# mazouziwissem/improving_yolov8_CBAM_SwinBlock

Hardware: AMD Instinct MI355X
Metric: images/sec fwd+bwd YOLOv8s-CBAM-Swin bs=32 640x640 (higher is better)
Workload: dtype bf16; 1 GPU; yolov8s.yaml (nc=1) forward + v8 loss + backward + clip + SGD-nesterov + EMA step, bs=32/GPU 640x640 (CBAM + 2x SwinBlock + SPPF5 + SPPF7); global_batch=32, imgsz=640, parallelism=dp1

## Files before the change

### improving_yolov8_cbam_swinblock_amd/csrc/common.h

```cpp
#pragma once
#include <hip/hip_runtime.h>
#include <stdint.h>
#include <stdio.h>

#include "../../include/ymi.h"

typedef __bf16 bf16_t;
typedef __attribute__((ext_vector_type(8))) __bf16 bf16x8;
typedef __attribute__((ext_vector_type(4))) __bf16 bf16x4;
typedef __attribute__((ext_vector_type(4))) float f32x4;
typedef __attribute__((ext_vector_type(2))) float f32x2;
typedef __attribute__((ext_vector_type(4))) uint32_t u32x4;
typedef __attribute__((ext_vector_type(2))) uint32_t u32x2;

typedef const __attribute__((address_space(1))) void* gptr_t;
typedef __attribute__((address_space(3))) void* lptr_t;

#define YMI_WAVE 64

void ymi_set_error(const char* fmt, ...);
#define YMI_CHECK_ARG(cond, ...)          \
    do {                                  \
        if (!(cond)) {                    \
            ymi_set_error(__VA_ARGS__);   \
            return YMI_EINVAL;            \
        }                                 \
    } while (0)
#define YMI_CHECK_LAUNCH(what)                                                   \
    do {                                                                         \
        hipError_t e_ = hipGetLastError();                                       \
        if (e_ != hipSuccess) {                                                  \
            ymi_set_error("%s: launch failed: %s", what, hipGetErrorString(e_)); \
            return YMI_ELAUNCH;                                                  \
        }                                                                        \
    } while (0)

static inline bool ymi_tensor_ok(const ymi_tensor* t) {
    return t && t->data && t->n > 0 && t->h > 0 && t->w > 0 && t->c > 0 && t->ld >= t->c && (t->dtype == YMI_F32 || t->dtype == YMI_BF16);
}
static inline int64_t ymi_pixels(const ymi_tensor* t) { return t->n * t->h * t->w; }
static inline int ymi_stat_fixed_point_shift(int64_t count) {
    int lg = 0;
    while (((int64_t)1 << lg) < count) ++lg;
    const int sh = 37 - lg;
    return sh < 8 ? 8 : sh > 40 ? 40 : sh;
}
static inline size_t ymi_esize(int dtype) { return dtype == YMI_BF16 ? 2 : 4; }
static inline bool ymi_same_shape(const ymi_tensor* a, const ymi_tensor* b) {
    return a->n == b->n && a->h == b->h && a->w == b->w && a->c == b->c;
}
enum YmiOpt {
    OPT_EW_PPT,
    OPT_EW_CAP,
    OPT_RED_CAP,
    OPT_XCD_SHIFT,
    OPT_ATTN_TILED,
    OPT_WGRAD_BLOCKS,
    OPT_WGRAD_BLOCKS128,
    OPT_IGEMM_TILE_BM,
    OPT_IGEMM_TILE_BN,
    OPT_BN_TAIL,
    OPT_WGRAD_PATCH,
    OPT_COUNT
};
int ymi_opt(int id);
static inline int ew_ppt() { return ymi_opt(OPT_EW_PPT); }
static inline int ew_cap() { return ymi_opt(OPT_EW_CAP); }
const void* ymi_zero_page();

template <typename T> struct ElemTraits;
template <> struct ElemTraits<float> {
    static constexpr int CH = 4;
    static constexpr int DT = YMI_F32;
};
template <> struct ElemTraits<bf16_t> {
    static constexpr int CH = 8;
    static constexpr int DT = YMI_BF16;
};

__device__ __forceinline__ float to_f32(float v) { return v; }
__device__ __forceinline__ float to_f32(bf16_t v) { return (float)v; }
template <typename T> __device__ __forceinline__ T from_f32(float v);
template <> __device__ __forceinline__ float from_f32<float>(float v) { return v; }
template <> __device__ __forceinline__ bf16_t from_f32<bf16_t>(float v) { return (bf16_t)v; }

template <typename T, int G> struct Pack;
template <> struct Pack<float, 4> {
    static __device__ __forceinline__ void load(const float* p, float (&v)[4]) {
        f32x4 t = *reinterpret_cast<const f32x4*>(p);
        v[0] = t[0]; v[1] = t[1]; v[2] = t[2]; v[3] = t[3];
    }
    static __device__ __forceinline__ void store(float* p, const float (&v)[4]) {
        f32x4 t = {v[0], v[1], v[2], v[3]};
        *reinterpret_cast<f32x4*>(p) = t;
    }
};
template <> struct Pack<bf16_t, 4> {
    static __device__ __forceinline__ void load(const bf16_t* p, float (&v)[4]) {
        bf16x4 t = *reinterpret_cast<const bf16x4*>(p);
        v[0] = (float)t[0]; v[1] = (float)t[1]; v[2] = (float)t[2]; v[3] = (float)t[3];
    }
    static __device__ __forceinline__ void store(bf16_t* p, const float (&v)[4]) {
        bf16x4 t = {(bf16_t)v[0], (bf16_t)v[1], (bf16_t)v[2], (bf16_t)v[3]};
        *reinterpret_cast<bf16x4*>(p) = t;
    }
};
template <> struct Pack<bf16_t, 8> {
    static __device__ __forceinline__ void load(const bf16_t* p, float (&v)[8]) {
        bf16x8 t = *reinterpret_cast<const bf16x8*>(p);
#pragma unroll
        for (int i = 0; i < 8; ++i) v[i] = (float)t[i];
    }
    static __device__ __forceinline__ void store(bf16_t* p, const float (&v)[8]) {
        bf16x8 t;
#pragma unroll
        for (int i = 0; i < 8; ++i) t[i] = (bf16_t)v[i];
        *reinterpret_cast<bf16x8*>(p) = t;
    }
};

template <typename T> struct Raw4;
template <> struct Raw4<bf16_t> {
    typedef bf16x4 type;
    static __device__ __forceinline__ void to_f32(const bf16x4& r, float (&v)[4]) {
#pragma unroll
        for (int i = 0; i < 4; ++i) v[i] = (float)r[i];
    }
};
template <> struct Raw4<float> {
    typedef f32x4 type;
    static __device__ __forceinline__ void to_f32(const f32x4& r, float (&v)[4]) {
#pragma unroll
        for (int i = 0; i < 4; ++i) v[i] = r[i];
    }
};

__host__ __device__ __forceinline__ int64_t ymi_xcd_span(int64_t P) { return (((P + 63) >> 6) + 7) >> 3 << 6; }
struct XcdRange {
    int64_t lo, hi;
    int bi, nbx;
};
int64_t ymi_xcd_span_arg(int64_t P);
__device__ __forceinline__ XcdRange xcd_range(int64_t P, int64_t span_arg) {
    const int id = blockIdx.x, x = ((id & 7) + (int)(span_arg >> 56)) & 7;
    const int64_t span = span_arg & ((1ll << 56) - 1);
// ... 220 lines not shown
```

### improving_yolov8_cbam_swinblock_amd/csrc/first_conv.hip

```cpp
#include "common.h"

namespace {

constexpr int FC_TH = 8, FC_TW = 64;
constexpr int FC_PR = 2 * FC_TH + 1;
constexpr int FC_ROWB = (2 * FC_TW + 2) * 8;
constexpr int FC_WG_TILES = 4;

enum { FC_STATS = 0, FC_APPLY = 1, FC_BWD_REDUCE = 2, FC_BWD_WGRAD = 3 };

struct FirstConvArgs {
    const float* img;
    const float* w;
    void* x4;
    void* out;
    int64_t ldout;
    float* partials;
    const float* v0;
    const float* v1;
    const float* v2;
    const float* v3;
    float* slab;
    int act;
    int N, C, H, W, Ho, Wo;
    int tiles_h, tiles_w, total;
};

template <int CTRL> __device__ __forceinline__ float fc_dpp_add(float v) {
    return v + __builtin_bit_cast(float, __builtin_amdgcn_update_dpp(0, __builtin_bit_cast(int, v), CTRL, 0xF, 0xF, true));
}
__device__ __forceinline__ float fc_row16_sum(float v) {
    v = fc_dpp_add<0xB1>(v);
    v = fc_dpp_add<0x4E>(v);
    v = fc_dpp_add<0x141>(v);
    v = fc_dpp_add<0x140>(v);
    return v;
}
__device__ __forceinline__ float fc_act(float x, int act) { return act == YMI_ACT_SILU ? silu_f(x) : x; }
__device__ __forceinline__ float fc_act_grad(float x, int act) { return act == YMI_ACT_SILU ? silu_grad_f(x) : 1.0f; }
__device__ __forceinline__ uint32_t fc_pack2(float lo, float hi) {
    typedef __attribute__((ext_vector_type(2))) __bf16 bf16x2;
    const bf16x2 v = {(bf16_t)lo, (bf16_t)hi};
    return __builtin_bit_cast(uint32_t, v);
}

template <int SW> __device__ __forceinline__ int fc_swz(int row) { return SW == 2 ? ((row >> 3) & 1) : (((row >> 1) & 1) | (((row >> 3) & 1) << 1)); }
template <int SW> __device__ __forceinline__ bf16x8 fc_tr_load(const char* img, int rowb, int c0, int lane) {
    typedef __attribute__((ext_vector_type(4))) short s16x4;
    typedef __attribute__((ext_vector_type(8))) short s16x8;
    const int g = lane >> 4, i = lane & 15, q = i >> 2, p = i & 3;
    const int r_lo = 8 * g + q, r_hi = r_lo + 4;
    const int u = (c0 >> 2) + p;
    const int u_lo = u ^ (fc_swz<SW>(r_lo) << 2), u_hi = u ^ (fc_swz<SW>(r_hi) << 2);
    const s16x4 lo = __builtin_amdgcn_ds_read_tr16_b64_v4i16((__attribute__((address_space(3))) s16x4*)(img + r_lo * rowb + u_lo * 8));
    const s16x4 hi = __builtin_amdgcn_ds_read_tr16_b64_v4i16((__attribute__((address_space(3))) s16x4*)(img + r_hi * rowb + u_hi * 8));
    const s16x8 v = {lo[0], lo[1], lo[2], lo[3], hi[0], hi[1], hi[2], hi[3]};
    return __builtin_bit_cast(bf16x8, v);
}

__device__ __forceinline__ void fc_patch_from_image(const FirstConvArgs& a, char* patch, int n, int oh0, int ow0, int tid) {
    const float* src = a.img + (int64_t)n * a.C * a.H * a.W;
    const int64_t plane = (int64_t)a.H * a.W;
    const int ih0 = 2 * oh0 - 1;
    constexpr int ITEMS = FC_PR * (2 * FC_TW / 4);
    constexpr int PASSES = (ITEMS + 255) / 256;
    f32x4 v[PASSES][3];
#pragma unroll
    for (int p = 0; p < PASSES; ++p) {
        const int it = tid + 256 * p;
        const int r = it / (2 * FC_TW / 4), g = it % (2 * FC_TW / 4);
        const int ih = ih0 + r, iw = 2 * ow0 + 4 * g;
        const bool ok = it < ITEMS && (unsigned)ih < (unsigned)a.H && iw < a.W;
#pragma unroll
        for (int c = 0; c < 3; ++c) v[p][c] = (ok && c < a.C) ? *reinterpret_cast<const f32x4*>(src + c * plane + (int64_t)ih * a.W + iw) : f32x4{0.f, 0.f, 0.f, 0.f};
    }
    float halo = 0.f;
    const int hr = tid / 4, hc = tid % 4;
    if (tid < FC_PR * 4) {
        const int ih = ih0 + hr, iw = 2 * ow0 - 1;
        if (hc < a.C && (unsigned)ih < (unsigned)a.H && iw >= 0) halo = src[hc * plane + (int64_t)ih * a.W + iw];
    }
#pragma unroll
    for (int p = 0; p < PASSES; ++p) {
        const int it = tid + 256 * p;
        if (it < ITEMS) {
            const int r = it / (2 * FC_TW / 4), g = it % (2 * FC_TW / 4);
            char* dst = patch + r * FC_ROWB + (4 * g + 2) * 8;
            *reinterpret_cast<u32x4*>(dst) = u32x4{fc_pack2(v[p][0][0], v[p][1][0]), fc_pack2(v[p][2][0], 0.f), fc_pack2(v[p][0][1], v[p][1][1]), fc_pack2(v[p][2][1], 0.f)};
            *reinterpret_cast<u32x4*>(dst + 16) = u32x4{fc_pack2(v[p][0][2], v[p][1][2]), fc_pack2(v[p][2][2], 0.f), fc_pack2(v[p][0][3], v[p][1][3]), fc_pack2(v[p][2][3], 0.f)};
        }
    }
    if (tid < FC_PR * 4) *reinterpret_cast<bf16_t*>(patch + hr * FC_ROWB + 1 * 8 + hc * 2) = (bf16_t)halo;
    if (a.C == 4) {
        __syncthreads();
        for (int e = tid; e < FC_PR * 2 * FC_TW; e += 256) {
            const int r = e / (2 * FC_TW), cc = e % (2 * FC_TW);
            const int ih = ih0 + r, iw = 2 * ow0 + cc;
            if ((unsigned)ih < (unsigned)a.H && iw < a.W) *reinterpret_cast<bf16_t*>(patch + r * FC_ROWB + (cc + 2) * 8 + 6) = (bf16_t)src[3 * plane + (int64_t)ih * a.W + iw];
        }
    }
    __syncthreads();
    bf16_t* x4 = reinterpret_cast<bf16_t*>(a.x4);
#pragma unroll 4
    for (int e = tid; e < 2 * FC_TH * FC_TW; e += 256) {
        const int r = e / FC_TW, cc = 2 * (e - r * FC_TW);
        const int ih = 2 * oh0 + r, iw = 2 * ow0 + cc;
        if (ih < a.H && iw < a.W) *reinterpret_cast<u32x4*>(x4 + (((int64_t)n * a.H + ih) * a.W + iw) * 4) = *reinterpret_cast<const u32x4*>(patch + (r + 1) * FC_ROWB + (cc + 2) * 8);
    }
}
__device__ __forceinline__ void fc_patch_from_x4(const FirstConvArgs& a, char* patch, int n, int oh0, int ow0, int tid) {
    const bf16_t* x4 = reinterpret_cast<const bf16_t*>(a.x4);
    const int ih0 = 2 * oh0 - 1;
    constexpr int ITEMS = FC_PR * FC_TW;
    constexpr int PASSES = (ITEMS + 255) / 256;
    u32x4 v[PASSES];
#pragma unroll
    for (int p = 0; p < PASSES; ++p) {
        const int it = tid + 256 * p;
        const int r = it / FC_TW, g = it % FC_TW;
        const int ih = ih0 + r, iw = 2 * ow0 + 2 * g;
        const bool ok = it < ITEMS && (unsigned)ih < (unsigned)a.H && iw < a.W;
        v[p] = ok ? *reinterpret_cast<const u32x4*>(x4 + (((int64_t)n * a.H + ih) * a.W + iw) * 4) : u32x4{0u, 0u, 0u, 0u};
    }
    u32x2 halo = u32x2{0u, 0u};
    if (tid < FC_PR) {
        const int ih = ih0 + tid, iw = 2 * ow0 - 1;
        if ((unsigned)ih < (unsigned)a.H && iw >= 0) halo = *reinterpret_cast<const u32x2*>(x4 + (((int64_t)n * a.H + ih) * a.W + iw) * 4);
    }
#pragma unroll
    for (int p = 0; p < PASSES; ++p) {
        const int it = tid + 256 * p;
        if (it < ITEMS) *reinterpret_cast<u32x4*>(patch + (it / FC_TW) * FC_ROWB + (2 * (it % FC_TW) + 2) * 8) = v[p];
    }
    if (tid < FC_PR) *reinterpret_cast<u32x2*>(patch + tid * FC_ROWB + 8) = halo;
    __syncthreads();
}

template <int NCT>
__device__ __forceinline__ void fc_conv_group(const char* patch, int ohl, int mt, int l15, int l4, const bf16x8 (&wf)[NCT][2], f32x4 (&acc)[NCT]) {
    const int owl = mt * 16 + l15;
    const int q0 = 2 * l4, q1 = 2 * l4 + 1;
    const u32x2 lo0 = *reinterpret_cast<const u32x2*>(patch + (2 * ohl + q0 / 3) * FC_ROWB + (2 * owl + q0 % 3 + 1) * 8);
    const u32x2 hi0 = *reinterpret_cast<const u32x2*>(patch + (2 * ohl + q1 / 3) * FC_ROWB + (2 * owl + q1 % 3 + 1) * 8);
    u32x2 lo1 = u32x2{0u, 0u};
    if (l4 == 0) lo1 = *reinterpret_cast<const u32x2*>(patch + (2 * ohl + 2) * FC_ROWB + (2 * owl + 2 + 1) * 8);
    const bf16x8 x0 = __builtin_bit_cast(bf16x8, u32x4{lo0[0], lo0[1], hi0[0], hi0[1]});
    const bf16x8 x1 = __builtin_bit_cast(bf16x8, u32x4{lo1[0], lo1[1], 0u, 0u});
#pragma unroll
    for (int ct = 0; ct < NCT; ++ct) {
        acc[ct] = __builtin_amdgcn_mfma_f32_16x16x32_bf16(wf[ct][0], x0, f32x4{0.f, 0.f, 0.f, 0.f}, 0, 0, 0);
        acc[ct] = __builtin_amdgcn_mfma_f32_16x16x32_bf16(wf[ct][1], x1, acc[ct], 0, 0, 0);
    }
}

template <int CO, int MODE>
__global__ __launch_bounds__(256, 4) void first_conv_kernel(FirstConvArgs a) {
    constexpr int NCT = CO / 16;
    constexpr int OUTB = FC_TW * CO * 2;
    constexpr int CPP = CO / 8;
    constexpr int DROWB = CO <= 32 ? 64 : 128, DSW = CO <= 32 ? 2 : 0;
    constexpr int STAGEB = MODE == FC_BWD_WGRAD ? FC_TW * DROWB : OUTB;
    __shared__ __attribute__((aligned(16))) char patch[FC_PR * FC_ROWB];
    __shared__ __attribute__((aligned(16))) char stage[(MODE == FC_APPLY || MODE == FC_BWD_WGRAD) ? 4 * STAGEB : 16];
    __shared__ __attribute__((aligned(16))) bf16_t wtab[CO * 64];
    __shared__ __attribute__((aligned(16))) float ctab[5 * CO];
    __shared__ float red[(MODE == FC_BWD_WGRAD) ? 48 * CO : 4 * 2 * CO];
    const int tid = threadIdx.x, lane = tid & 63, wave = tid >> 6;
    const int l15 = lane & 15, l4 = lane >> 4;

#pragma unroll
    for (int i = 0; i < CO * 64 / 256; ++i) {
        const int e = tid + 256 * i, co = e >> 6, k = e & 63, q = k >> 2, c = k & 3;
        wtab[e] = (bf16_t)((q < 9 && c < a.C) ? a.w[(co * a.C + c) * 9 + q] : 0.f);
    }
    if (tid < CO) {
        float c0 = 0.f, c1 = 0.f, c2 = 0.f, c3 = 0.f, c4 = 0.f;
        if constexpr (MODE == FC_APPLY) {
            c0 = a.v0[tid];
            c1 = a.v1[tid];
        } else if constexpr (MODE == FC_BWD_REDUCE) {
            const float g = a.v0 ? a.v0[tid] : 1.f, bb = a.v1 ? a.v1[tid] : 0.f, mu = a.v2[tid], iv = a.v3[tid];
            c0 = iv;
            c1 = -mu * iv;
            c2 = g;
            c3 = bb;
        } else if constexpr (MODE == FC_BWD_WGRAD) {
            c0 = a.v0[tid];
            c1 = a.v0[CO + tid];
            c2 = a.v0[2 * CO + tid];
            c3 = a.v0[3 * CO + tid];
            c4 = a.v0[4 * CO + tid];
        }
        ctab[tid] = c0; ctab[CO + tid] = c1; ctab[2 * CO + tid] = c2; ctab[3 * CO + tid] = c3; ctab[4 * CO + tid] = c4;
    }
    __syncthreads();
    bf16x8 wf[NCT][2];
#pragma unroll
    for (int ct = 0; ct < NCT; ++ct)
#pragma unroll
        for (int h = 0; h < 2; ++h) wf[ct][h] = *reinterpret_cast<const bf16x8*>(wtab + (ct * 16 + l15) * 64 + 32 * h + 8 * l4);

    float s1[NCT][4], s2[NCT][4];
#pragma unroll
    for (int ct = 0; ct < NCT; ++ct)
#pragma unroll
        for (int r = 0; r < 4; ++r) s1[ct][r] = s2[ct][r] = 0.f;
    f32x4 dwa[3][NCT];
#pragma unroll
    for (int kt = 0; kt < 3; ++kt)
#pragma unroll
        for (int ct = 0; ct < NCT; ++ct) dwa[kt][ct] = f32x4{0.f, 0.f, 0.f, 0.f};

    char* my = stage + ((MODE == FC_APPLY || MODE == FC_BWD_WGRAD) ? wave * STAGEB : 0);
    constexpr int TILES = MODE == FC_BWD_WGRAD ? FC_WG_TILES : 1;
    const int wg_unit = xcd_unit(blockIdx.x, gridDim.x);
#pragma unroll 1
    for (int ti = 0; ti < TILES; ++ti) {
        const int unit = wg_unit * TILES + ti;
        if (unit >= a.total) break;
        const int tw = unit % a.tiles_w;
        const int t2 = unit / a.tiles_w;
        const int th = t2 % a.tiles_h, n = t2 / a.tiles_h;
        const int oh0 = th * FC_TH, ow0 = tw * FC_TW;
        if (ti > 0) __syncthreads();
        if constexpr (MODE == FC_STATS) fc_patch_from_image(a, patch, n, oh0, ow0, tid);
        else fc_patch_from_x4(a, patch, n, oh0, ow0, tid);

#pragma unroll 1
        for (int rr = 0; rr < FC_TH / 4; ++rr) {
            const int ohl = wave + 4 * rr;
            const int oh = oh0 + ohl;
            const bool row_ok = oh < a.Ho;
            const int64_t rowbase = (((int64_t)n * a.Ho + oh) * a.Wo + ow0) * a.ldout;
            [[maybe_unused]] bf16x4 dy_cur[NCT], dy_nxt[NCT];
            [[maybe_unused]] auto load_dy = [&](int mt, bf16x4 (&dst)[NCT]) {
                const bf16_t* dyp = reinterpret_cast<const bf16_t*>(a.out);
                const int owl = mt * 16 + l15;
                const bool ok = row_ok && ow0 + owl < a.Wo;
#pragma unroll
                for (int ct = 0; ct < NCT; ++ct)
                    dst[ct] = ok ? *reinterpret_cast<const bf16x4*>(dyp + rowbase + (int64_t)owl * a.ldout + ct * 16 + 4 * l4) : bf16x4{(bf16_t)0.f, (bf16_t)0.f, (bf16_t)0.f, (bf16_t)0.f};
            };
            if constexpr (MODE == FC_BWD_REDUCE || MODE == FC_BWD_WGRAD) load_dy(0, dy_cur);
#pragma unroll 1
            for (int mt = 0; mt < 4; ++mt) {
                const int owl = mt * 16 + l15;
                const bool ok = row_ok && ow0 + owl < a.Wo;
                if constexpr (MODE == FC_BWD_REDUCE || MODE == FC_BWD_WGRAD) {
                    if (mt + 1 < 4) load_dy(mt + 1, dy_nxt);
                }
                f32x4 acc[NCT];
                fc_conv_group<NCT>(patch, ohl, mt, l15, l4, wf, acc);
#pragma unroll
                for (int ct = 0; ct < NCT; ++ct) {
                    int ch0 = ct * 16 + 4 * l4;
                    asm volatile("" : "+v"(ch0));
                    float raw[4];
#pragma unroll
                    for (int r = 0; r < 4; ++r) raw[r] = (float)(bf16_t)acc[ct][r];
                    if constexpr (MODE == FC_STATS) {
#pragma unroll
                        for (int r = 0; r < 4; ++r) {
                            const float v = ok ? raw[r] : 0.f;
                            s1[ct][r] += v;
                            s2[ct][r] += v * v;
                        }
                    } else if constexpr (MODE == FC_APPLY) {
                        const f32x4 sc = *reinterpret_cast<const f32x4*>(ctab + ch0), sh = *reinterpret_cast<const f32x4*>(ctab + CO + ch0);
                        bf16x4 o;
#pragma unroll
                        for (int r = 0; r < 4; ++r) o[r] = (bf16_t)fc_act(raw[r] * sc[r] + sh[r], a.act);
                        *reinterpret_cast<bf16x4*>(my + (owl * CO + ch0) * 2) = o;
                    } else if constexpr (MODE == FC_BWD_REDUCE) {
                        const f32x4 iv = *reinterpret_cast<const f32x4*>(ctab + ch0), of = *reinterpret_cast<const f32x4*>(ctab + CO + ch0);
                        const f32x4 g = *reinterpret_cast<const f32x4*>(ctab + 2 * CO + ch0), bb = *reinterpret_cast<const f32x4*>(ctab + 3 * CO + ch0);
#pragma unroll
                        for (int r = 0; r < 4; ++r) {
                            const float xh = raw[r] * iv[r] + of[r];
                            const float dz = (float)dy_cur[ct][r] * fc_act_grad(xh * g[r] + bb[r], a.act);
                            s1[ct][r] += dz;
                            s2[ct][r] += dz * xh;
                        }
                    } else {
                        const f32x4 a0 = *reinterpret_cast<const f32x4*>(ctab + ch0), a1 = *reinterpret_cast<const f32x4*>(ctab + CO + ch0);
// ... 13 lines not shown
                    for (int ct = 0; ct < NCT; ++ct) dy_cur[ct] = dy_nxt[ct];
                }
            }
            if constexpr (MODE == FC_APPLY) {
                if (row_ok) {
                    bf16_t* outp = reinterpret_cast<bf16_t*>(a.out);
#pragma unroll
                    for (int it = 0; it < FC_TW * CPP / 64; ++it) {
                        const int q = it * 64 + lane;
                        const int px = q / CPP, cc = q % CPP;
                        if (ow0 + px < a.Wo) *reinterpret_cast<u32x4*>(outp + rowbase + (int64_t)px * a.ldout + cc * 8) = *reinterpret_cast<const u32x4*>(my + q * 16);
                    }
                }
            } else if constexpr (MODE == FC_BWD_WGRAD) {
#pragma unroll
                for (int h = 0; h < 2; ++h) {
                    bf16x8 df[NCT];
#pragma unroll
                    for (int ct = 0; ct < NCT; ++ct) df[ct] = fc_tr_load<DSW>(my + 32 * h * DROWB, DROWB, ct * 16, lane);
#pragma unroll
                    for (int kt = 0; kt < 3; ++kt) {
                        const int k = kt * 16 + l15, q = k >> 2, c = k & 3;
                        bf16x8 xf;
                        if (q < 9) {
                            const char* base = patch + (2 * ohl + q / 3) * FC_ROWB + (q % 3 + 1) * 8 + c * 2 + (32 * h + 8 * l4) * 16;
#pragma unroll
                            for (int j = 0; j < 8; ++j) xf[j] = *reinterpret_cast<const bf16_t*>(base + j * 16);
                        } else {
#pragma unroll
                            for (int j = 0; j < 8; ++j) xf[j] = (bf16_t)0.f;
                        }
#pragma unroll
                        for (int ct = 0; ct < NCT; ++ct) dwa[kt][ct] = __builtin_amdgcn_mfma_f32_16x16x32_bf16(xf, df[ct], dwa[kt][ct], 0, 0, 0);
                    }
                }
            }
        }
        if constexpr (MODE == FC_STATS || MODE == FC_BWD_REDUCE) {
#pragma unroll
            for (int ct = 0; ct < NCT; ++ct)
#pragma unroll
                for (int r = 0; r < 4; ++r) {
                    const float t1 = fc_row16_sum(s1[ct][r]), t2s = fc_row16_sum(s2[ct][r]);
                    if (l15 == 0) {
                        red[(wave * 2 + 0) * CO + ct * 16 + 4 * l4 + r] = t1;
                        red[(wave * 2 + 1) * CO + ct * 16 + 4 * l4 + r] = t2s;
                    }
                }
            __syncthreads();
            if (tid < 2 * CO) {
                const int which = tid / CO, ch = tid % CO;
                a.partials[((int64_t)unit * 2 + which) * CO + ch] = (red[(0 * 2 + which) * CO + ch] + red[(1 * 2 + which) * CO + ch]) + (red[(2 * 2 + which) * CO + ch] + red[(3 * 2 + which) * CO + ch]);
            }
        }
    }
    if constexpr (MODE == FC_BWD_WGRAD) {
        for (int wv = 0; wv < 4; ++wv) {
            if (wave == wv) {
#pragma unroll
                for (int kt = 0; kt < 3; ++kt)
#pragma unroll
                    for (int ct = 0; ct < NCT; ++ct)
#pragma unroll
                        for (int r = 0; r < 4; ++r) {
                            float* dst = &red[(kt * 16 + 4 * l4 + r) * CO + ct * 16 + l15];
                            *dst = wv == 0 ? dwa[kt][ct][r] : *dst + dwa[kt][ct][r];
                        }
            }
            __syncthreads();
        }
        float* slab = a.slab + (int64_t)wg_unit * CO * 72;
        for (int e = tid; e < CO * 72; e += 256) {
            const int co = e / 72, col = e % 72, tap = col >> 3, c = col & 7;
            slab[e] = c < 4 ? red[(tap * 4 + c) * CO + co] : 0.f;
        }
    }
}

template <int MODE>
int fc_launch(const FirstConvArgs& a, int64_t cout, unsigned blocks, hipStream_t s) {
    dim3 grid(blocks), blk(256);
    if (cout == 16) hipLaunchKernelGGL((first_conv_kernel<16, MODE>), grid, blk, 0, s, a);
    else if (cout == 32) hipLaunchKernelGGL((first_conv_kernel<32, MODE>), grid, blk, 0, s, a);
    else if (cout == 48) hipLaunchKernelGGL((first_conv_kernel<48, MODE>), grid, blk, 0, s, a);
    else hipLaunchKernelGGL((first_conv_kernel<64, MODE>), grid, blk, 0, s, a);
    YMI_CHECK_LAUNCH("first_conv");
    return YMI_OK;
}

int fc_geometry(FirstConvArgs& a, int64_t n, int64_t c, int64_t h, int64_t w, int64_t cout) {
    YMI_CHECK_ARG(c >= 1 && c <= 4 && (cout == 16 || cout == 32 || cout == 48 || cout == 64), "first_conv: c <= 4 input channels, 16 / 32 / 48 / 64 output channels");
    YMI_CHECK_ARG(a.act == YMI_ACT_SILU || a.act == YMI_ACT_NONE, "first_conv: SiLU or no activation");
    YMI_CHECK_ARG(w % 4 == 0 && h % 2 == 0 && n > 0, "first_conv: even height, width a multiple of 4");
    const int64_t ho = h / 2, wo = w / 2;
    YMI_CHECK_ARG(n * ho * wo * cout < (1ll << 31) && n * h * w * 4 < (1ll << 31), "first_conv: too large for 32-bit indexing");
    a.N = (int)n; a.C = (int)c; a.H = (int)h; a.W = (int)w; a.Ho = (int)ho; a.Wo = (int)wo;
    a.tiles_h = (int)((ho + FC_TH - 1) / FC_TH); a.tiles_w = (int)((wo + FC_TW - 1) / FC_TW);
    a.total = (int)(n * a.tiles_h * a.tiles_w);
    return YMI_OK;
}

}

extern "C" int64_t ymi_first_conv_stat_blocks(int64_t n, int64_t h, int64_t w) {
    const int64_t ho = h / 2, wo = w / 2;
    return n * ((ho + FC_TH - 1) / FC_TH) * ((wo + FC_TW - 1) / FC_TW);
}

extern "C" int ymi_first_conv_bn_act_fwd(const float* img_nchw, int64_t n, int64_t c, int64_t h, int64_t w, const float* weight_oihw, int64_t cout,
                                         const float* gamma, const float* beta, float* running_mean, float* running_var, float momentum, float eps,
                                         int32_t act, const ymi_tensor* x4, const ymi_tensor* out, float* save_mean, float* save_invstd,
                                         void* workspace, size_t workspace_bytes, void* stream) {
    YMI_CHECK_ARG(img_nchw && weight_oihw && ymi_tensor_ok(out) && ymi_tensor_ok(x4) && workspace, "first_conv: bad argument");
    YMI_CHECK_ARG(((uintptr_t)img_nchw & 15) == 0, "first_conv: 16-byte aligned image");
    FirstConvArgs a{};
    a.act = act;
    int rc = fc_geometry(a, n, c, h, w, cout);
    if (rc) return rc;
    YMI_CHECK_ARG(out->dtype == YMI_BF16 && out->n == n && out->h == a.Ho && out->w == a.Wo && out->c == cout && out->ld % 8 == 0 && ((uintptr_t)out->data & 15) == 0,
                  "first_conv: output must be bfloat16 [n, cout, h/2, w/2] NHWC with 16-byte aligned rows");
    YMI_CHECK_ARG(x4->dtype == YMI_BF16 && x4->n == n && x4->h == h && x4->w == w && x4->c == 4 && x4->ld == 4 && ((uintptr_t)x4->data & 15) == 0,
                  "first_conv: the image copy must be dense bfloat16 [n, 4, h, w] NHWC");
    const int64_t blocks = a.total;
    const size_t need = (size_t)(2 * cout + (blocks + 64) * 2 * cout) * sizeof(float);
    if (workspace_bytes < need) {
        ymi_set_error("first_conv: workspace %zu < %zu bytes", workspace_bytes, need);
        return YMI_EWORKSPACE;
    }
    float* scale = reinterpret_cast<float*>(workspace);
    float* shift = scale + cout;
    a.img = img_nchw; a.w = weight_oihw; a.x4 = x4->data; a.partials = shift + cout;
    hipStream_t s = (hipStream_t)stream;
    rc = fc_launch<FC_STATS>(a, cout, (unsigned)blocks, s);
    if (rc) return rc;
    rc = ymi_bn_finalize(a.partials, blocks, n * a.Ho * a.Wo, cout, gamma, beta, running_mean, running_var, momentum, eps, scale, shift, save_mean, save_invstd, stream);
    if (rc) return rc;
    a.out = out->data; a.ldout = out->ld; a.v0 = scale; a.v1 = shift;
    return fc_launch<FC_APPLY>(a, cout, (unsigned)blocks, s);
}

extern "C" int64_t ymi_first_conv_bwd_workspace(int64_t n, int64_t h, int64_t w, int64_t cout) {
    const int64_t blocks = ymi_first_conv_stat_blocks(n, h, w), wgs = (blocks + FC_WG_TILES - 1) / FC_WG_TILES;
    return (int64_t)sizeof(float) * (blocks * 2 * cout + 5 * cout + wgs * cout * 72) + 1024;
}

extern "C" int ymi_first_conv_bn_act_bwd(const ymi_tensor* x4, const float* weight_oihw, int64_t c, int64_t cout, const float* gamma, const float* beta,
                                         const float* save_mean, const float* save_invstd, int32_t act, const ymi_tensor* dout, float* dgamma,
                                         float* dbeta, float* dw_oihw, void* workspace, size_t workspace_bytes, ymi_wgrad_pending* pending, void* stream) {
    YMI_CHECK_ARG(ymi_tensor_ok(x4) && ymi_tensor_ok(dout) && weight_oihw && save_mean && save_invstd && dgamma && dbeta && dw_oihw && workspace, "first_conv_bwd: bad argument");
    FirstConvArgs a{};
    a.act = act;
    int rc = fc_geometry(a, x4->n, c, x4->h, x4->w, cout);
    if (rc) return rc;
    YMI_CHECK_ARG(x4->dtype == YMI_BF16 && x4->c == 4 && x4->ld == 4 && ((uintptr_t)x4->data & 15) == 0, "first_conv_bwd: the image copy must be dense bfloat16 [n, 4, h, w] NHWC");
    YMI_CHECK_ARG(dout->dtype == YMI_BF16 && dout->n == x4->n && dout->h == a.Ho && dout->w == a.Wo && dout->c == cout && dout->ld % 4 == 0 && ((uintptr_t)dout->data & 7) == 0,
                  "first_conv_bwd: dout must be bfloat16 [n, cout, h/2, w/2] NHWC");
    const int64_t blocks = a.total, wgs = (blocks + FC_WG_TILES - 1) / FC_WG_TILES;
    if ((int64_t)workspace_bytes < ymi_first_conv_bwd_workspace(x4->n, x4->h, x4->w, cout)) {
        ymi_set_error("first_conv_bwd: workspace too small");
        return YMI_EWORKSPACE;
    }
    float* part = reinterpret_cast<float*>(workspace);
    float* coef = part + blocks * 2 * cout;
    float* slab = coef + 5 * cout;
    ymi_wgrad_pending* table = reinterpret_cast<ymi_wgrad_pending*>(slab + wgs * cout * 72);
    table = reinterpret_cast<ymi_wgrad_pending*>(((uintptr_t)table + 63) & ~(uintptr_t)63);
    hipStream_t s = (hipStream_t)stream;
    a.w = weight_oihw; a.x4 = x4->data; a.out = dout->data; a.ldout = dout->ld;
    a.partials = part; a.v0 = gamma; a.v1 = beta; a.v2 = save_mean; a.v3 = save_invstd;
    rc = fc_launch<FC_BWD_REDUCE>(a, cout, (unsigned)blocks, s);
    if (rc) return rc;
    rc = ymi_bn_bwd_final(part, (int)blocks, (int)cout, gamma, beta, save_mean, save_invstd, 1.0f / (float)((int64_t)x4->n * a.Ho * a.Wo), dgamma, dbeta, coef, s);
    if (rc) return rc;
    a.v0 = coef; a.slab = slab;
    rc = fc_launch<FC_BWD_WGRAD>(a, cout, (unsigned)wgs, s);
    if (rc) return rc;
    const int64_t elems = cout * 72;
    const int lanes = wgs > 128 ? 32 : wgs > 32 ? 16 : wgs > 8 ? 8 : 4;
    ymi_wgrad_pending rec{slab, dw_oihw, elems, (int32_t)wgs, 72, 8, (int32_t)cout, (int32_t)c, 9, lanes, 0, (int32_t)((elems / 4 + 256 / lanes - 1) / (256 / lanes)), 0};
    if (pending) {
        *pending = rec;
        return YMI_OK;
    }
    return ymi_wgrad_reduce_batch(&rec, 1, table, stream);
}
```

### improving_yolov8_cbam_swinblock_amd/csrc/runtime.hip

```cpp
#include <stdarg.h>
#include <string.h>

#include <stdlib.h>

#include "common.h"

static thread_local char g_err[512] = "";

void ymi_set_error(const char* fmt, ...) {
    va_list ap;
    va_start(ap, fmt);
    vsnprintf(g_err, sizeof(g_err), fmt, ap);
    va_end(ap);
}

extern "C" int ymi_version(void) { return YMI_VERSION; }
extern "C" const char* ymi_last_error(void) { return g_err; }

__device__ __attribute__((aligned(256))) unsigned char ymi_zero_page_storage[256];

const void* ymi_zero_page() {
    static thread_local int cached_dev = -1;
    static thread_local void* cached_ptr = nullptr;
    int dev = 0;
    if (hipGetDevice(&dev) != hipSuccess) return nullptr;
    if (dev != cached_dev) {
        void* p = nullptr;
        if (hipGetSymbolAddress(&p, HIP_SYMBOL(ymi_zero_page_storage)) != hipSuccess) return nullptr;
        cached_ptr = p;
        cached_dev = dev;
    }
    return cached_ptr;
}

struct OptEntry {
    const char* name;
    int value;
};
static OptEntry g_opts[OPT_COUNT] = {
    {"ew_ppt", 64}, {"ew_cap", 512}, {"red_cap", 512}, {"xcd_shift", 0}, {"attn_tiled", 0}, {"wgrad_blocks", 1280}, {"wgrad_blocks128", 768},
    {"igemm_tile_bm", 0}, {"igemm_tile_bn", 0}, {"bn_tail", 0}, {"wgrad_patch", 1},
};
static void opts_from_env() {
    for (int i = 0; i < OPT_COUNT; ++i) {
        char env[64] = "YMI_";
        size_t n = 4;
        for (const char* c = g_opts[i].name; *c && n + 1 < sizeof(env); ++c) env[n++] = (char)((*c >= 'a' && *c <= 'z') ? *c - 32 : *c);
        env[n] = 0;
        if (const char* v = getenv(env)) g_opts[i].value = atoi(v);
    }
    if (const char* t = getenv("YMI_IGEMM_TILE")) {
        int bm = 0, bn = 0;
        if (sscanf(t, "%d,%d", &bm, &bn) == 2) {
            g_opts[OPT_IGEMM_TILE_BM].value = bm;
            g_opts[OPT_IGEMM_TILE_BN].value = bn;
        }
    }
}
int ymi_opt(int id) {
    static const bool init = (opts_from_env(), true);
    (void)init;
    return g_opts[id].value;
}
extern "C" int ymi_set_option(const char* name, int64_t value) {
    (void)ymi_opt(0);
    for (int i = 0; name && i < OPT_COUNT; ++i)
        if (!strcmp(name, g_opts[i].name)) {
            g_opts[i].value = (int)value;
            return YMI_OK;
        }
    ymi_set_error("set_option: unknown option '%s'", name ? name : "(null)");
    return YMI_EINVAL;
}
extern "C" int64_t ymi_get_option(const char* name) {
    (void)ymi_opt(0);
    for (int i = 0; name && i < OPT_COUNT; ++i)
        if (!strcmp(name, g_opts[i].name)) return g_opts[i].value;
    ymi_set_error("get_option: unknown option '%s'", name ? name : "(null)");
    return -1;
}

int64_t ymi_xcd_span_arg(int64_t P) { return ymi_xcd_span(P) | ((int64_t)(ymi_opt(OPT_XCD_SHIFT) & 7) << 56); }

__device__ unsigned ymi_ticket_storage[1024 * 64];
unsigned* ymi_ticket_slot() {
    static thread_local int cached_dev = -1;
    static thread_local unsigned* base = nullptr;
    static unsigned counter = 0;
    int dev = 0;
    if (hipGetDevice(&dev) != hipSuccess) return nullptr;
    if (dev != cached_dev) {
        void* p = nullptr;
        if (hipGetSymbolAddress(&p, HIP_SYMBOL(ymi_ticket_storage)) != hipSuccess) return nullptr;
        base = (unsigned*)p;
        cached_dev = dev;
    }
    return base + (size_t)(__atomic_fetch_add(&counter, 1u, __ATOMIC_RELAXED) % 1024u) * 64;
}
```

Before: 2726 images/sec.

## Fuse first-conv BN backward reduce and weight-grad into one pass

Adds a one-pass backward for the stem conv with BN+SiLU (up to 32 output channels). It recomputes the conv output once, accumulates the BN sums together with three separate weight-gradient terms (dz*x, raw*x, x) via MFMA, and combines them in a final kernel using the BN coefficients algebraically. This replaces the two passes over the input and dout (reduce, then wgrad) with one, at the cost of extra MFMA work, a hi/lo bf16 split of dz for precision, and a double-precision final combine. Launch bounds for several modes also change.

New measurement: 2748 images/sec (median of 6 runs). Within noise of the previous version (+0.8%).

```diff
diff --git a/improving_yolov8_cbam_swinblock_amd/csrc/common.h b/improving_yolov8_cbam_swinblock_amd/csrc/common.h
--- a/improving_yolov8_cbam_swinblock_amd/csrc/common.h
+++ b/improving_yolov8_cbam_swinblock_amd/csrc/common.h
@@ -61,6 +61,7 @@
     OPT_IGEMM_TILE_BN,
     OPT_BN_TAIL,
     OPT_WGRAD_PATCH,
+    OPT_FIRST_CONV_ONE_PASS,
     OPT_COUNT
 };
 int ymi_opt(int id);
diff --git a/improving_yolov8_cbam_swinblock_amd/csrc/first_conv.hip b/improving_yolov8_cbam_swinblock_amd/csrc/first_conv.hip
--- a/improving_yolov8_cbam_swinblock_amd/csrc/first_conv.hip
+++ b/improving_yolov8_cbam_swinblock_amd/csrc/first_conv.hip
@@ -7,7 +7,10 @@
 constexpr int FC_ROWB = (2 * FC_TW + 2) * 8;
 constexpr int FC_WG_TILES = 4;
 
-enum { FC_STATS = 0, FC_APPLY = 1, FC_BWD_REDUCE = 2, FC_BWD_WGRAD = 3 };
+enum { FC_STATS = 0, FC_APPLY = 1, FC_BWD_REDUCE = 2, FC_BWD_WGRAD = 3, FC_BWD_ONE = 4 };
+constexpr int FC_ONE_MAX_WGS = 512;
+constexpr int FC_ONE_IMGB = 32 * 64;
+constexpr int64_t fc_one_set(int64_t co) { return 2 * co * 72 + 72 + 2 * co; }
 
 struct FirstConvArgs {
     const float* img;
@@ -21,6 +24,7 @@
     const float* v2;
     const float* v3;
     float* slab;
+    int tiles_per_wg;
     int act;
     int N, C, H, W, Ho, Wo;
     int tiles_h, tiles_w, total;
@@ -108,12 +112,18 @@
         if (ih < a.H && iw < a.W) *reinterpret_cast<u32x4*>(x4 + (((int64_t)n * a.H + ih) * a.W + iw) * 4) = *reinterpret_cast<const u32x4*>(patch + (r + 1) * FC_ROWB + (cc + 2) * 8);
     }
 }
-__device__ __forceinline__ void fc_patch_from_x4(const FirstConvArgs& a, char* patch, int n, int oh0, int ow0, int tid) {
+constexpr int FC_X4_ITEMS = FC_PR * FC_TW;
+constexpr int FC_X4_PASSES = (FC_X4_ITEMS + 255) / 256;
+struct FcX4Regs {
+    u32x4 v[FC_X4_PASSES];
+    u32x2 halo;
+};
+__device__ __forceinline__ void fc_x4_fetch(const FirstConvArgs& a, int n, int oh0, int ow0, int tid, FcX4Regs& x) {
     const bf16_t* x4 = reinterpret_cast<const bf16_t*>(a.x4);
     const int ih0 = 2 * oh0 - 1;
-    constexpr int ITEMS = FC_PR * FC_TW;
-    constexpr int PASSES = (ITEMS + 255) / 256;
-    u32x4 v[PASSES];
+    constexpr int ITEMS = FC_X4_ITEMS, PASSES = FC_X4_PASSES;
+    u32x4 (&v)[PASSES] = x.v;
+    u32x2& halo = x.halo;
 #pragma unroll
     for (int p = 0; p < PASSES; ++p) {
         const int it = tid + 256 * p;
@@ -122,18 +132,25 @@
         const bool ok = it < ITEMS && (unsigned)ih < (unsigned)a.H && iw < a.W;
         v[p] = ok ? *reinterpret_cast<const u32x4*>(x4 + (((int64_t)n * a.H + ih) * a.W + iw) * 4) : u32x4{0u, 0u, 0u, 0u};
     }
-    u32x2 halo = u32x2{0u, 0u};
+    halo = u32x2{0u, 0u};
     if (tid < FC_PR) {
         const int ih = ih0 + tid, iw = 2 * ow0 - 1;
         if ((unsigned)ih < (unsigned)a.H && iw >= 0) halo = *reinterpret_cast<const u32x2*>(x4 + (((int64_t)n * a.H + ih) * a.W + iw) * 4);
     }
-#pragma unroll
-    for (int p = 0; p < PASSES; ++p) {
+}
+__device__ __forceinline__ void fc_x4_put(char* patch, int tid, const FcX4Regs& x) {
+#pragma unroll
+    for (int p = 0; p < FC_X4_PASSES; ++p) {
         const int it = tid + 256 * p;
-        if (it < ITEMS) *reinterpret_cast<u32x4*>(patch + (it / FC_TW) * FC_ROWB + (2 * (it % FC_TW) + 2) * 8) = v[p];
-    }
-    if (tid < FC_PR) *reinterpret_cast<u32x2*>(patch + tid * FC_ROWB + 8) = halo;
+        if (it < FC_X4_ITEMS) *reinterpret_cast<u32x4*>(patch + (it / FC_TW) * FC_ROWB + (2 * (it % FC_TW) + 2) * 8) = x.v[p];
+    }
+    if (tid < FC_PR) *reinterpret_cast<u32x2*>(patch + tid * FC_ROWB + 8) = x.halo;
     __syncthreads();
+}
+__device__ __forceinline__ void fc_patch_from_x4(const FirstConvArgs& a, char* patch, int n, int oh0, int ow0, int tid) {
+    FcX4Regs x;
+    fc_x4_fetch(a, n, oh0, ow0, tid, x);
+    fc_x4_put(patch, tid, x);
 }
 
 template <int NCT>
@@ -153,18 +170,288 @@
     }
 }
 
+
+template <int CO>
+__device__ __forceinline__ void fc_bwd_one_pass(const FirstConvArgs& a, char* patch, char* stage, const float* ctab, float* red, const bf16x8 (&wf)[CO / 16][2]) {
+    constexpr int NCT = CO / 16;
+    const int tid = threadIdx.x, lane = tid & 63, wave = tid >> 6;
+    const int l15 = lane & 15, l4 = lane >> 4;
+    char* my = stage + wave * 3 * FC_ONE_IMGB;
+    float s1[NCT][4], s2[NCT][4];
+    f32x4 sa[3][NCT], sb[3][NCT], sc[3];
+#pragma unroll
+    for (int ct = 0; ct < NCT; ++ct)
+#pragma unroll
+        for (int r = 0; r < 4; ++r) s1[ct][r] = s2[ct][r] = 0.f;
+#pragma unroll
+    for (int kt = 0; kt < 3; ++kt) {
+        sc[kt] = f32x4{0.f, 0.f, 0.f, 0.f};
+#pragma unroll
+        for (int ct = 0; ct < NCT; ++ct) sa[kt][ct] = sb[kt][ct] = f32x4{0.f, 0.f, 0.f, 0.f};
+    }
+    const int wg_unit = xcd_unit(blockIdx.x, gridDim.x);
+    const int u0 = wg_unit * a.tiles_per_wg;
+    const int u1 = u0 + a.tiles_per_wg < a.total ? u0 + a.tiles_per_wg : a.total;
+    struct Tile { int n, oh0, ow0; };
+    auto tile_of = [&](int unit) {
+        const int tw = unit % a.tiles_w, t2 = unit / a.tiles_w;
+        return Tile{t2 / a.tiles_h, (t2 % a.tiles_h) * FC_TH, tw * FC_TW};
+    };
+    auto load_half = [&](int hq, bf16x4 (&dst)[2][NCT]) {
+        const bf16_t* dyp = reinterpret_cast<const bf16_t*>(a.out);
+        const int unit = u0 + (hq >> 2);
+        const Tile t = tile_of(unit);
+        const int oh = t.oh0 + wave + 4 * ((hq >> 1) & 1);
+        const int64_t rowbase = (((int64_t)t.n * a.Ho + oh) * a.Wo + t.ow0) * a.ldout;
+#pragma unroll
+        for (int mi = 0; mi < 2; ++mi) {
+            const int owl = 32 * (hq & 1) + mi * 16 + l15;
+            const bool ok = unit < u1 && oh < a.Ho && t.ow0 + owl < a.Wo;
+#pragma unroll
+            for (int ct = 0; ct < NCT; ++ct)
+                dst[mi][ct] = ok ? *reinterpret_cast<const bf16x4*>(dyp + rowbase + (int64_t)owl * a.ldout + ct * 16 + 4 * l4) : bf16x4{(bf16_t)0.f, (bf16_t)0.f, (bf16_t)0.f, (bf16_t)0.f};
+        }
+    };
+    FcX4Regs px;
+    bf16x4 dy[2][NCT], dy1[2][NCT], dy2[2][NCT];
+    if (u0 < u1) {
+        const Tile t = tile_of(u0);
+        fc_x4_fetch(a, t.n, t.oh0, t.ow0, tid, px);
+    }
+    load_half(0, dy);
+    load_half(1, dy1);
+#pragma unroll 1
+    for (int unit = u0; unit < u1; ++unit) {
+        const Tile t = tile_of(unit);
+        if (unit > u0) __syncthreads();
+        fc_x4_put(patch, tid, px);
+        if (unit + 1 < u1) {
+            const Tile tn = tile_of(unit + 1);
+            fc_x4_fetch(a, tn.n, tn.oh0, tn.ow0, tid, px);
+        }
+#pragma unroll 1
+        for (int q = 0; q < 4; ++q) {
+            const int h = q & 1;
+            const int ohl = wave + 4 * (q >> 1);
+            const bool row_ok = t.oh0 + ohl < a.Ho;
+            load_half(4 * (unit - u0) + q + 2, dy2);
+#pragma unroll
+            for (int mi = 0; mi < 2; ++mi) {
+                const int mt = 2 * h + mi;
+                const int owl = mt * 16 + l15;
+                const bool ok = row_ok && t.ow0 + owl < a.Wo;
+                f32x4 acc[NCT];
+                fc_conv_group<NCT>(patch, ohl, mt, l15, l4, wf, acc);
+#pragma unroll
+                for (int ct = 0; ct < NCT; ++ct) {
+                    int ch0 = ct * 16 + 4 * l4;
+                    asm volatile("" : "+v"(ch0));
+                    const f32x4 iv = *reinterpret_cast<const f32x4*>(ctab + ch0), of = *reinterpret_cast<const f32x4*>(ctab + CO + ch0);
+                    const f32x4 g = *reinterpret_cast<const f32x4*>(ctab + 2 * CO + ch0), bb = *reinterpret_cast<const f32x4*>(ctab + 3 * CO + ch0);
+                    bf16x4 hi, lo, rw;
+#pragma unroll
+                    for (int r = 0; r < 4; ++r) {
+                        const float raw = (float)(bf16_t)acc[ct][r];
+                        const float xh = raw * iv[r] + of[r];
+                        const float dz = (float)dy[mi][ct][r] * fc_act_grad(xh * g[r] + bb[r], a.act);
+                        s1[ct][r] += dz;
+                        s2[ct][r] += dz * xh;
+                        hi[r] = (bf16_t)dz;
+                        lo[r] = (bf16_t)(dz - (float)hi[r]);
+                        rw[r] = (bf16_t)(ok ? raw : 0.f);
+                    }
+                    char* dst = my + (owl & 31) * 64 + ((ch0 >> 2) ^ (fc_swz<2>(owl & 31) << 2)) * 8;
+                    *reinterpret_cast<bf16x4*>(dst) = hi;
+                    *reinterpret_cast<bf16x4*>(dst + FC_ONE_IMGB) = lo;
+                    *reinterpret_cast<bf16x4*>(dst + 2 * FC_ONE_IMGB) = rw;
+                }
+            }
+            {
+                bf16x8 fh[NCT], fl[NCT], fr[NCT], one;
+#pragma unroll
+                for (int ct = 0; ct < NCT; ++ct) {
+                    fh[ct] = fc_tr_load<2>(my, 64, ct * 16, lane);
+                    fl[ct] = fc_tr_load<2>(my + FC_ONE_IMGB, 64, ct * 16, lane);
+                    fr[ct] = fc_tr_load<2>(my + 2 * FC_ONE_IMGB, 64, ct * 16, lane);
+                }
+#pragma unroll
+                for (int j = 0; j < 8; ++j) one[j] = (bf16_t)((row_ok && t.ow0 + 32 * h + 8 * l4 + j < a.Wo) ? 1.f : 0.f);
+#pragma unroll
+                for (int kt = 0; kt < 3; ++kt) {
+                    const int k = kt * 16 + l15, q = k >> 2, c = k & 3;
+                    bf16x8 xf;
+                    if (q < 9) {
+                        const char* base = patch + (2 * ohl + q / 3) * FC_ROWB + (q % 3 + 1) * 8 + c * 2 + (32 * h + 8 * l4) * 16;
+#pragma unroll
+                        for (int j = 0; j < 8; ++j) xf[j] = *reinterpret_cast<const bf16_t*>(base + j * 16);
+                    } else {
+#pragma unroll
+                        for (int j = 0; j < 8; ++j) xf[j] = (bf16_t)0.f;
+                    }
+#pragma unroll
+                    for (int ct = 0; ct < NCT; ++ct) {
+                        sa[kt][ct] = __builtin_amdgcn_mfma_f32_16x16x32_bf16(xf, fh[ct], sa[kt][ct], 0, 0, 0);
+                        sa[kt][ct] = __builtin_amdgcn_mfma_f32_16x16x32_bf16(xf, fl[ct], sa[kt][ct], 0, 0, 0);
+                        sb[kt][ct] = __builtin_amdgcn_mfma_f32_16x16x32_bf16(xf, fr[ct], sb[kt][ct], 0, 0, 0);
+                    }
+                    sc[kt] = __builtin_amdgcn_mfma_f32_16x16x32_bf16(xf, one, sc[kt], 0, 0, 0);
+                }
+            }
+#pragma unroll
+            for (int mi = 0; mi < 2; ++mi)
+#pragma unroll
+                for (int ct = 0; ct < NCT; ++ct) {
+                    dy[mi][ct] = dy1[mi][ct];
+                    dy1[mi][ct] = dy2[mi][ct];
+                }
+        }
+    }
+    float* set = a.slab + (int64_t)wg_unit * fc_one_set(CO);
+    __syncthreads();
+#pragma unroll
+    for (int ct = 0; ct < NCT; ++ct)
+#pragma unroll
+        for (int r = 0; r < 4; ++r) {
+            const float t1 = fc_row16_sum(s1[ct][r]), t2s = fc_row16_sum(s2[ct][r]);
+            if (l15 == 0) {
+                red[(wave * 2 + 0) * CO + ct * 16 + 4 * l4 + r] = t1;
+                red[(wave * 2 + 1) * CO + ct * 16 + 4 * l4 + r] = t2s;
+            }
+        }
+    __syncthreads();
+    if (tid < 2 * CO) {
+        const int which = tid / CO, ch = tid % CO;
+        set[2 * CO * 72 + 72 + tid] = (red[(0 * 2 + which) * CO + ch] + red[(1 * 2 + which) * CO + ch]) + (red[(2 * 2 + which) * CO + ch] + red[(3 * 2 + which) * CO + ch]);
+    }
+    __syncthreads();
+#pragma unroll
+    for (int m = 0; m < 2; ++m) {
+        for (int wv = 0; wv < 4; ++wv) {
+            if (wave == wv) {
+#pragma unroll
+                for (int kt = 0; kt < 3; ++kt)
+#pragma unroll
+                    for (int ct = 0; ct < NCT; ++ct)
+#pragma unroll
+                        for (int r = 0; r < 4; ++r) {
+                            float* dst = &red[(kt * 16 + 4 * l4 + r) * CO + ct * 16 + l15];
+                            const float v = m == 0 ? sa[kt][ct][r] : sb[kt][ct][r];
+                            *dst = wv == 0 ? v : *dst + v;
+                        }
+            }
+            __syncthreads();
+        }
+        for (int e = tid; e < CO * 72; e += 256) {
+            const int co = e / 72, col = e % 72, tap = col >> 3, c = col & 7;
+            set[m * CO * 72 + e] = c < 4 ? red[(tap * 4 + c) * CO + co] : 0.f;
+        }
+        __syncthreads();
+    }
+    for (int wv = 0; wv < 4; ++wv) {
+        if (wave == wv && l15 == 0) {
+#pragma unroll
+            for (int kt = 0; kt < 3; ++kt)
+#pragma unroll
+                for (int r = 0; r < 4; ++r) {
+                    float* dst = &red[kt * 16 + 4 * l4 + r];
+                    *dst = wv == 0 ? sc[kt][r] : *dst + sc[kt][r];
+                }
+        }
+        __syncthreads();
+    }
+    if (tid < 72) set[2 * CO * 72 + tid] = (tid & 7) < 4 ? red[(tid >> 3) * 4 + (tid & 7)] : 0.f;
+}
+
+struct FcOneFinal {
+    const float* sets;
+    int wgs, C;
+    const float* gamma;
+    const float* beta;
+    const float* mean;
+    const float* inv;
+    float inv_count;
+    float* dgamma;
+    float* dbeta;
+    float* slab;
+};
+constexpr int FC_FIN_SLICES = 14;
+__global__ __launch_bounds__(1024) void fc_bwd_one_final_kernel(FcOneFinal f) {
+    __shared__ double red[2 * FC_ONE_MAX_WGS];
+    __shared__ double red2[2 * 32];
+    __shared__ double tot[2];
+    __shared__ double part[3 * FC_FIN_SLICES * 72];
+    const int tid = threadIdx.x, co = blockIdx.x, C = f.C;
+    const int64_t setf = fc_one_set(C);
+    const int col = tid % 72, slice = tid / 72;
+    double p1 = 0.0, p2 = 0.0, p3 = 0.0;
+    if (slice < FC_FIN_SLICES) {
+        const float* base = f.sets + (int64_t)co * 72 + col;
+#pragma unroll 4
+        for (int k = slice; k < f.wgs; k += FC_FIN_SLICES) {
+            const float* sp = base + (int64_t)k * setf;
+            p1 += (double)sp[0];
+            p2 += (double)sp[(int64_t)C * 72];
+            p3 += (double)f.sets[(int64_t)k * setf + 2 * C * 72 + col];
+        }
+        part[(0 * FC_FIN_SLICES + slice) * 72 + col] = p1;
+        part[(1 * FC_FIN_SLICES + slice) * 72 + col] = p2;
+        part[(2 * FC_FIN_SLICES + slice) * 72 + col] = p3;
+    }
+    {
+        const int which = tid & 1, k = tid >> 1;
+        red[which * FC_ONE_MAX_WGS + k] = k < f.wgs ? (double)f.sets[(int64_t)k * setf + 2 * C * 72 + 72 + which * C + co] : 0.0;
+    }
+    __syncthreads();
+    if (tid < 64) {
+        const int which = tid >> 5, j = tid & 31;
+        double s = 0.0;
+#pragma unroll
+        for (int i = 0; i < FC_ONE_MAX_WGS / 32; ++i) s += red[which * FC_ONE_MAX_WGS + j * (FC_ONE_MAX_WGS / 32) + i];
+        red2[which * 32 + j] = s;
+    }
+    __syncthreads();
+    if (tid < 2) {
+        double s = 0.0;
+        for (int j = 0; j < 32; ++j) s += red2[tid * 32 + j];
+        tot[tid] = s;
+    }
+    __syncthreads();
+    const float s0 = (float)tot[0], s1 = (float)tot[1];
+    if (tid == 0) {
+        f.dbeta[co] = s0;
+        f.dgamma[co] = s1;
+    }
+    if (tid < 72) {
+        const float ga = f.gamma ? f.gamma[co] : 1.0f;
+        const float p0 = f.inv[co], pm = -f.mean[co] * p0;
+        const float k1 = s0 * f.inv_count, k2 = s1 * f.inv_count;
+        const float c0 = ga * p0, c1 = ga * p0 * p0 * k2, c2 = ga * p0 * (k1 + pm * k2);
+        double a1 = 0.0, a2 = 0.0, a3 = 0.0;
+#pragma unroll
+        for (int q = 0; q < FC_FIN_SLICES; ++q) {
+            a1 += part[(0 * FC_FIN_SLICES + q) * 72 + tid];
+            a2 += part[(1 * FC_FIN_SLICES + q) * 72 + tid];
+            a3 += part[(2 * FC_FIN_SLICES + q) * 72 + tid];
+        }
+        f.slab[(int64_t)co * 72 + tid] = (float)((double)c0 * a1 - (double)c1 * a2 - (double)c2 * a3);
+    }
+}
+
+constexpr int fc_waves(int co, int mode) {
+    return mode == FC_BWD_ONE ? 2 : mode == FC_APPLY ? (co == 64 ? 2 : co == 48 ? 3 : 4) : mode == FC_BWD_WGRAD ? (co >= 48 ? 2 : co == 32 ? 3 : 4) : 4;
+}
 template <int CO, int MODE>
-__global__ __launch_bounds__(256, 4) void first_conv_kernel(FirstConvArgs a) {
+__global__ __launch_bounds__(256, fc_waves(CO, MODE)) void first_conv_kernel(FirstConvArgs a) {
     constexpr int NCT = CO / 16;
     constexpr int OUTB = FC_TW * CO * 2;
     constexpr int CPP = CO / 8;
     constexpr int DROWB = CO <= 32 ? 64 : 128, DSW = CO <= 32 ? 2 : 0;
-    constexpr int STAGEB = MODE == FC_BWD_WGRAD ? FC_TW * DROWB : OUTB;
+    constexpr int STAGEB = MODE == FC_BWD_ONE ? 3 * FC_ONE_IMGB : MODE == FC_BWD_WGRAD ? FC_TW * DROWB : OUTB;
     __shared__ __attribute__((aligned(16))) char patch[FC_PR * FC_ROWB];
-    __shared__ __attribute__((aligned(16))) char stage[(MODE == FC_APPLY || MODE == FC_BWD_WGRAD) ? 4 * STAGEB : 16];
+    __shared__ __attribute__((aligned(16))) char stage[(MODE == FC_APPLY || MODE == FC_BWD_WGRAD || MODE == FC_BWD_ONE) ? 4 * STAGEB : 16];
     __shared__ __attribute__((aligned(16))) bf16_t wtab[CO * 64];
     __shared__ __attribute__((aligned(16))) float ctab[5 * CO];
-    __shared__ float red[(MODE == FC_BWD_WGRAD) ? 48 * CO : 4 * 2 * CO];
+    __shared__ float red[(MODE == FC_BWD_WGRAD || MODE == FC_BWD_ONE) ? 48 * CO : 4 * 2 * CO];
     const int tid = threadIdx.x, lane = tid & 63, wave = tid >> 6;
     const int l15 = lane & 15, l4 = lane >> 4;
 
@@ -178,7 +465,7 @@
         if constexpr (MODE == FC_APPLY) {
             c0 = a.v0[tid];
             c1 = a.v1[tid];
-        } else if constexpr (MODE == FC_BWD_REDUCE) {
+        } else if constexpr (MODE == FC_BWD_REDUCE || MODE == FC_BWD_ONE) {
             const float g = a.v0 ? a.v0[tid] : 1.f, bb = a.v1 ? a.v1[tid] : 0.f, mu = a.v2[tid], iv = a.v3[tid];
             c0 = iv;
             c1 = -mu * iv;
@@ -200,6 +487,11 @@
 #pragma unroll
         for (int h = 0; h < 2; ++h) wf[ct][h] = *reinterpret_cast<const bf16x8*>(wtab + (ct * 16 + l15) * 64 + 32 * h + 8 * l4);
 
+    if constexpr (MODE == FC_BWD_ONE) {
+        static_assert(MODE != FC_BWD_ONE || CO <= 32, "S1 + S2 at 64 channels are 96 accumulator registers: wider layers keep the two passes");
+        fc_bwd_one_pass<CO>(a, patch, stage, ctab, red, wf);
+        return;
+    }
     float s1[NCT][4], s2[NCT][4];
 #pragma unroll
     for (int ct = 0; ct < NCT; ++ct)
@@ -379,6 +671,7 @@
     dim3 grid(blocks), blk(256);
     if (cout == 16) hipLaunchKernelGGL((first_conv_kernel<16, MODE>), grid, blk, 0, s, a);
     else if (cout == 32) hipLaunchKernelGGL((first_conv_kernel<32, MODE>), grid, blk, 0, s, a);
+    else if constexpr (MODE == FC_BWD_ONE) YMI_CHECK_ARG(false, "first_conv: the one-pass backward takes at most 32 output channels");
     else if (cout == 48) hipLaunchKernelGGL((first_conv_kernel<48, MODE>), grid, blk, 0, s, a);
     else hipLaunchKernelGGL((first_conv_kernel<64, MODE>), grid, blk, 0, s, a);
     YMI_CHECK_LAUNCH("first_conv");
@@ -436,9 +729,18 @@
     return fc_launch<FC_APPLY>(a, cout, (unsigned)blocks, s);
 }
 
+static int64_t fc_one_wgs(int64_t blocks, int64_t* per) {
+    *per = (blocks + FC_ONE_MAX_WGS - 1) / FC_ONE_MAX_WGS;
+    if (*per < FC_WG_TILES) *per = FC_WG_TILES;
+    return ((blocks + *per - 1) / *per + 7) / 8 * 8;
+}
+static bool fc_one_pass(int64_t cout) { return cout <= 32 && ymi_opt(OPT_FIRST_CONV_ONE_PASS) != 0; }
+
 extern "C" int64_t ymi_first_conv_bwd_workspace(int64_t n, int64_t h, int64_t w, int64_t cout) {
     const int64_t blocks = ymi_first_conv_stat_blocks(n, h, w), wgs = (blocks + FC_WG_TILES - 1) / FC_WG_TILES;
-    return (int64_t)sizeof(float) * (blocks * 2 * cout + 5 * cout + wgs * cout * 72) + 1024;
+    int64_t per;
+    const int64_t two = blocks * 2 * cout + 5 * cout + wgs * cout * 72, one = fc_one_wgs(blocks, &per) * fc_one_set(cout) + cout * 72;
+    return (int64_t)sizeof(float) * (two > one ? two : one) + 1024;
 }
 
 extern "C" int ymi_first_conv_bn_act_bwd(const ymi_tensor* x4, const float* weight_oihw, int64_t c, int64_t cout, const float* gamma, const float* beta,
@@ -457,22 +759,43 @@
         ymi_set_error("first_conv_bwd: workspace too small");
         return YMI_EWORKSPACE;
     }
+    hipStream_t s = (hipStream_t)stream;
+    a.w = weight_oihw; a.x4 = x4->data; a.out = dout->data; a.ldout = dout->ld;
+    a.v0 = gamma; a.v1 = beta; a.v2 = save_mean; a.v3 = save_invstd;
+    const float inv_count = 1.0f / (float)((int64_t)x4->n * a.Ho * a.Wo);
+    const int64_t elems = cout * 72;
+    if (fc_one_pass(cout)) {
+        int64_t per;
+        const int64_t owgs = fc_one_wgs(blocks, &per);
+        float* sets = reinterpret_cast<float*>(workspace);
+        float* comb = sets + owgs * fc_one_set(cout);
+        ymi_wgrad_pending* table = reinterpret_cast<ymi_wgrad_pending*>(((uintptr_t)(comb + elems) + 63) & ~(uintptr_t)63);
+        a.slab = sets; a.tiles_per_wg = (int)per;
+        rc = fc_launch<FC_BWD_ONE>(a, cout, (unsigned)owgs, s);
+        if (rc) return rc;
+        hipLaunchKernelGGL(fc_bwd_one_final_kernel, dim3((unsigned)cout), dim3(1024), 0, s,
+                           FcOneFinal{sets, (int)owgs, (int)cout, gamma, beta, save_mean, save_invstd, inv_count, dgamma, dbeta, comb});
+        YMI_CHECK_LAUNCH("first_conv_bwd_final");
+        ymi_wgrad_pending rec{comb, dw_oihw, elems, 1, 72, 8, (int32_t)cout, (int32_t)c, 9, 4, 0, (int32_t)((elems / 4 + 256 / 4 - 1) / (256 / 4)), 0};
+        if (pending) {
+            *pending = rec;
+            return YMI_OK;
+        }
+        return ymi_wgrad_reduce_batch(&rec, 1, table, stream);
+    }
     float* part = reinterpret_cast<float*>(workspace);
     float* coef = part + blocks * 2 * cout;
     float* slab = coef + 5 * cout;
     ymi_wgrad_pending* table = reinterpret_cast<ymi_wgrad_pending*>(slab + wgs * cout * 72);
     table = reinterpret_cast<ymi_wgrad_pending*>(((uintptr_t)table + 63) & ~(uintptr_t)63);
-    hipStream_t s = (hipStream_t)stream;
-    a.w = weight_oihw; a.x4 = x4->data; a.out = dout->data; a.ldout = dout->ld;
-    a.partials = part; a.v0 = gamma; a.v1 = beta; a.v2 = save_mean; a.v3 = save_invstd;
+    a.partials = part;
     rc = fc_launch<FC_BWD_REDUCE>(a, cout, (unsigned)blocks, s);
     if (rc) return rc;
-    rc = ymi_bn_bwd_final(part, (int)blocks, (int)cout, gamma, beta, save_mean, save_invstd, 1.0f / (float)((int64_t)x4->n * a.Ho * a.Wo), dgamma, dbeta, coef, s);
+    rc = ymi_bn_bwd_final(part, (int)blocks, (int)cout, gamma, beta, save_mean, save_invstd, inv_count, dgamma, dbeta, coef, s);
     if (rc) return rc;
     a.v0 = coef; a.slab = slab;
     rc = fc_launch<FC_BWD_WGRAD>(a, cout, (unsigned)wgs, s);
     if (rc) return rc;
-    const int64_t elems = cout * 72;
     const int lanes = wgs > 128 ? 32 : wgs > 32 ? 16 : wgs > 8 ? 8 : 4;
     ymi_wgrad_pending rec{slab, dw_oihw, elems, (int32_t)wgs, 72, 8, (int32_t)cout, (int32_t)c, 9, lanes, 0, (int32_t)((elems / 4 + 256 / lanes - 1) / (256 / lanes)), 0};
     if (pending) {
diff --git a/improving_yolov8_cbam_swinblock_amd/csrc/runtime.hip b/improving_yolov8_cbam_swinblock_amd/csrc/runtime.hip
--- a/improving_yolov8_cbam_swinblock_amd/csrc/runtime.hip
+++ b/improving_yolov8_cbam_swinblock_amd/csrc/runtime.hip
@@ -39,7 +39,7 @@
 };
 static OptEntry g_opts[OPT_COUNT] = {
     {"ew_ppt", 64}, {"ew_cap", 512}, {"red_cap", 512}, {"xcd_shift", 0}, {"attn_tiled", 0}, {"wgrad_blocks", 1280}, {"wgrad_blocks128", 768},
-    {"igemm_tile_bm", 0}, {"igemm_tile_bn", 0}, {"bn_tail", 0}, {"wgrad_patch", 1},
+    {"igemm_tile_bm", 0}, {"igemm_tile_bn", 0}, {"bn_tail", 0}, {"wgrad_patch", 1}, {"first_conv_one_pass", 1},
 };
 static void opts_from_env() {
     for (int i = 0; i < OPT_COUNT; ++i) {
```
